# OATML/oatomobile

Hardware: AMD Instinct MI355X
Metric: RIPAgent.act() calls/sec (K=4, 128 plans, 200x200 BEV) (higher is better)
Workload: dtype bf16 encoder (bf16 storage, fp32 accumulate) + flow/search: fp32 accumulate, GRU/head contractions as two-term binary16 (22-bit) operands on f16 MFMA (the waypoint / bias terms as three-term, 33-bit operands); 1 GPU; BASELINE configs[2]: RIPAgent K=4 WCM, N=128 candidate plans, 10 Adam steps, 200x200x2 BEV, bf16 encoder + fp32 flow; models=4, candidates=128, bev_channels=2, parallelism=observation-parallel replicas x1 (no data-path collective)

## Files before the change

oatomobile_amd/csrc/encoder_bf16_tile.hip:

```cpp
#include <cstdio>

#include "encoder.h"
#include "flow.h"

namespace rip {

namespace {

using f32x4 = __attribute__((ext_vector_type(4))) float;
using f32x2 = __attribute__((ext_vector_type(2))) float;
using bf16x8 = __attribute__((ext_vector_type(8))) __bf16;
using bf16x2 = __attribute__((ext_vector_type(2))) __bf16;
using u32x4 = __attribute__((ext_vector_type(4))) unsigned int;
using u32x2 = __attribute__((ext_vector_type(2))) unsigned int;
typedef unsigned short bf16_t;

__device__ __forceinline__ bf16x8 as_bf16x8(u32x4 u) {
  union {
    u32x4 u;
    bf16x8 v;
  } c;
  c.u = u;
  return c.v;
}
__device__ __forceinline__ f32x2 bfpair(unsigned u) {
  f32x2 r;
  r.x = __uint_as_float(u << 16);
  r.y = __uint_as_float(u & 0xffff0000u);
  return r;
}
__device__ __forceinline__ unsigned pack_bf16(f32x2 v) {
  union {
    bf16x2 h;
    unsigned u;
  } c;
  c.h = __builtin_convertvector(v, bf16x2);
  return c.u;
}
__device__ __forceinline__ f32x2 relu6_2(f32x2 v) {
  return __builtin_elementwise_min(__builtin_elementwise_max(v, f32x2{0.f, 0.f}), f32x2{6.f, 6.f});
}

#ifndef RIP_TILE_ABL
#define RIP_TILE_ABL 0
#endif

#ifdef RIP_TILE_TICKS
__device__ unsigned long long g_tile_ticks[16];
#define TILE_TICK(slot_)                                            \
  do {                                                              \
    const unsigned long long now_ = __builtin_readcyclecounter();   \
    tk[slot_] += now_ - tlast;                                      \
    tlast = now_;                                                   \
  } while (0)
#else
#define TILE_TICK(slot_) do { } while (0)
#endif

constexpr int HC = 64;
constexpr int LD = HC + 8;

struct TileArgs {
  const bf16_t* x;
  bf16_t* y;
  const float* wbase;
  const bf16_t* whbase;
  size_t model_stride;
  int k0;
  size_t we_off, be_off, wd_off, bd_off, wp_off, bp_off;
  int B, HID, residual, G;
};

template <int HIN, int STRIDE, int G>
struct TileGeom {
  static constexpr int HOUT = STRIDE == 1 ? HIN : (HIN + 1) / 2;
  static constexpr int HWI = HIN * HIN, HWO = HOUT * HOUT;
  static constexpr int PW = HIN + 2;
  static constexpr int E_DUMP = G * HIN * PW;
  static constexpr int E_ROWS = E_DUMP + 1;
  static constexpr int D_ROWS = ((G * HWO + 15) / 16) * 16;
  static constexpr int TIN = (G * HWI + 63) / 64, TOUT = (G * HWO + 63) / 64;
  static constexpr size_t ED_BYTES = (size_t)2 * (E_ROWS + D_ROWS) * LD * sizeof(bf16_t);
  static constexpr size_t lds_bytes(int hid) { return ED_BYTES + (size_t)10 * hid * sizeof(float); }
};

template <int HIN, int STRIDE, int CIN, int COUT, int G, bool AEF, bool APF, int WCH = 1>
__global__ __launch_bounds__(512) void irb_tile_bf16_kernel(TileArgs a) {
  using Geo = TileGeom<HIN, STRIDE, G>;
  constexpr int HOUT = Geo::HOUT, HWI = Geo::HWI, HWO = Geo::HWO, PW = Geo::PW;
  constexpr int WP = 4 / WCH;
  constexpr int TIN = (Geo::TIN * 4 + WP - 1) / WP, TOUT = (Geo::TOUT * 4 + WP - 1) / WP;
  constexpr int KSX = CIN / 32, NCT = COUT / 16 / WCH, NHT = HC / 16 / WCH, NKP = HC / 32;
  static_assert((COUT / 16) % WCH == 0 && (HC / 16) % WCH == 0, "channel partitions");
  constexpr int NPT_IN = (G * HWI + 15) / 16, NPT_OUT = (G * HWO + 15) / 16;
  constexpr int CTG = NCT > 10 ? 10 : NCT;
  static_assert(NCT % CTG == 0 && (CTG == NCT || !APF), "projection passes");
  extern __shared__ __attribute__((aligned(16))) unsigned char smem_raw[];
  bf16_t* const Ebuf = reinterpret_cast<bf16_t*>(smem_raw);
  bf16_t* const Dbuf = Ebuf + (size_t)2 * Geo::E_ROWS * LD;
  float* const Tl = reinterpret_cast<float*>(smem_raw + Geo::ED_BYTES);
  const int tid = threadIdx.x, lane = tid & 63;
  const int w = __builtin_amdgcn_readfirstlane(tid >> 6);
  const int k = blockIdx.z;
  const int HID = a.HID;
  const int nch = HID / HC;
  const float* W = a.wbase + (size_t)(a.k0 + k) * a.model_stride;
  const bf16_t* Wh = a.whbase + (size_t)(a.k0 + k) * a.model_stride;
  const u32x4 zero4 = {0u, 0u, 0u, 0u};
  const int n_groups = (a.B + a.G - 1) / a.G;
  const int ng = (n_groups - 1 - (int)blockIdx.x) / (int)gridDim.x + 1;
  int img0 = 0, m_in = 0, m_out = 0;
  const bf16_t* xg = nullptr;
  bf16_t* yg = nullptr;
  auto enter_group = [&](int j) {
    img0 = ((int)blockIdx.x + j * (int)gridDim.x) * a.G;
    const int n_img = min(a.G, a.B - img0);
    m_in = n_img * HWI;
    m_out = n_img * HWO;
    xg = a.x + ((size_t)k * a.B + img0) * HWI * CIN;
    yg = a.y + ((size_t)k * a.B + img0) * HWO * COUT;
  };

#ifdef RIP_TILE_TICKS
  unsigned long long tk[10] = {0, 0, 0, 0, 0, 0, 0, 0, 0, 0};
  unsigned long long tlast = __builtin_readcyclecounter();
#endif
  if (!(RIP_TILE_ABL & 8))
    for (int e = tid; e < 2 * Geo::E_ROWS * LD / 8; e += 512) reinterpret_cast<u32x4*>(Ebuf)[e] = zero4;
  {
    const int HIDs = a.HID;
    const float* Wk = a.wbase + (size_t)(a.k0 + blockIdx.z) * a.model_stride;
    for (int e = tid; e < 9 * HIDs / 4; e += 512)
      reinterpret_cast<float4*>(Tl)[e] = *reinterpret_cast<const float4*>(Wk + a.wd_off + 4 * e);
    for (int e = tid; e < HIDs / 4; e += 512)
      reinterpret_cast<float4*>(Tl + 9 * HIDs)[e] = *reinterpret_cast<const float4*>(Wk + a.bd_off + 4 * e);
  }
  lds_barrier();
  TILE_TICK(0);

  if (w < 4) {
    const int n = lane & 15, q = lane >> 4;
    const int wpix = w / WCH, wch = w % WCH;
    const int ht0 = wch * NHT, ct0w = wch * NCT;
    u32x4 xb[TIN][KSX];
    int erow[TIN];
    f32x4 acc[TOUT][NCT];

    u32x4 ae[NHT][KSX], ap[CTG][NKP];
    float4 be[NHT];
    auto load_ae = [&](int c) {
      int n_ = n, q_ = q;
      asm volatile("" : "+v"(n_), "+v"(q_));
#pragma unroll
      for (int ht = 0; ht < NHT; ++ht) {
#pragma unroll
        for (int ks = 0; ks < KSX; ++ks)
          ae[ht][ks] = *reinterpret_cast<const u32x4*>(Wh + a.we_off + (size_t)(c * HC + 16 * (ht0 + ht) + n_) * CIN + 32 * ks + 8 * q_);
        be[ht] = *reinterpret_cast<const float4*>(W + a.be_off + c * HC + 16 * (ht0 + ht) + 4 * q_);
      }
    };
    auto load_ap = [&](int c, int ct0) {
      int n_ = n, q_ = q;
      asm volatile("" : "+v"(n_), "+v"(q_));
      const bf16_t* wp = Wh + a.wp_off + (size_t)(16 * (ct0w + ct0) + n_) * HID + c * HC + 8 * q_;
#pragma unroll
      for (int ct = 0; ct < CTG; ++ct)
#pragma unroll
        for (int ks = 0; ks < NKP; ++ks) ap[ct][ks] = *reinterpret_cast<const u32x4*>(wp + (size_t)16 * ct * HID + 32 * ks);
    };
    auto tile_on = [&](int t, int npt) { return !(WP * t + WP - 1 >= npt && wpix + WP * t >= npt); };
    auto expand = [&](int c) {
      bf16_t* E = Ebuf + (size_t)(c & 1) * Geo::E_ROWS * LD;
      if (!AEF && !((RIP_TILE_ABL & 32) && c > 0)) load_ae(c);
      f32x4 v[2][NHT];
      auto mm = [&](int t, f32x4(&o)[NHT]) {
#pragma unroll
        for (int ht = 0; ht < NHT; ++ht) o[ht] = f32x4{0.f, 0.f, 0.f, 0.f};
#pragma unroll
        for (int ks = 0; ks < KSX; ++ks)
#pragma unroll
          for (int ht = 0; ht < NHT; ++ht)
            o[ht] = __builtin_amdgcn_mfma_f32_16x16x32_bf16(as_bf16x8(ae[ht][ks]), as_bf16x8(xb[t][ks]), o[ht], 0, 0, 0);
      };
      auto epi = [&](int t, const f32x4(&o)[NHT]) {
#pragma unroll
        for (int ht = 0; ht < NHT; ++ht) {
          u32x2 w2;
          w2.x = pack_bf16(relu6_2(f32x2{o[ht][0] + be[ht].x, o[ht][1] + be[ht].y}));
          w2.y = pack_bf16(relu6_2(f32x2{o[ht][2] + be[ht].z, o[ht][3] + be[ht].w}));
          *reinterpret_cast<u32x2*>(E + (size_t)erow[t] * LD + 16 * (ht0 + ht) + 4 * q) = w2;
        }
      };
      if (tile_on(0, NPT_IN)) mm(0, v[0]);
#pragma unroll
      for (int t = 0; t < TIN; ++t) {
        if (t + 1 < TIN && tile_on(t + 1, NPT_IN)) mm(t + 1, v[(t + 1) & 1]);
        if (tile_on(t, NPT_IN)) epi(t, v[t & 1]);
      }
      if (AEF && c + 1 < nch && !(RIP_TILE_ABL & 32)) load_ae(c + 1);
    };
    auto project = [&](int c) {
      const bf16_t* D = Dbuf + (size_t)(c & 1) * Geo::D_ROWS * LD;
#pragma unroll
      for (int cg = 0; cg < NCT; cg += CTG) {
        if (!APF && !((RIP_TILE_ABL & 32) && c > 0)) load_ap(c, cg);
        u32x4 bv[2][NKP];
        auto rd = [&](int t, u32x4(&o)[NKP]) {
#pragma unroll
          for (int ks = 0; ks < NKP; ++ks)
            o[ks] = *reinterpret_cast<const u32x4*>(D + (size_t)(16 * (wpix + WP * t) + n) * LD + 32 * ks + 8 * q);
        };
        if (tile_on(0, NPT_OUT)) rd(0, bv[0]);
#pragma unroll
        for (int t = 0; t < TOUT; ++t) {
          if (t + 1 < TOUT && tile_on(t + 1, NPT_OUT)) rd(t + 1, bv[(t + 1) & 1]);
          if (!tile_on(t, NPT_OUT)) continue;
#pragma unroll
          for (int ks = 0; ks < NKP; ++ks)
#pragma unroll
            for (int ct = 0; ct < CTG; ++ct)
              acc[t][cg + ct] = __builtin_amdgcn_mfma_f32_16x16x32_bf16(as_bf16x8(ap[ct][ks]), as_bf16x8(bv[t & 1][ks]), acc[t][cg + ct], 0, 0, 0);
        }
      }
      if (APF && c + 1 < nch && !(RIP_TILE_ABL & 32)) load_ap(c + 1, 0);
    };
    const bool mx_on = !(RIP_TILE_ABL & 2);
#pragma unroll 1
    for (int j = 0; j < ng; ++j) {
    enter_group(j);
    int ng_ = n, qg_ = q;
    asm volatile("" : "+v"(ng_), "+v"(qg_));
#pragma unroll
    for (int t = 0; t < TIN; ++t) {
      const int px = 16 * (wpix + WP * t) + ng_;
#pragma unroll
      for (int ks = 0; ks < KSX; ++ks)
        xb[t][ks] = px < m_in ? *reinterpret_cast<const u32x4*>(xg + (size_t)px * CIN + 32 * ks + 8 * qg_) : zero4;
      const int g = px / HWI, r = px - g * HWI, iy = r / HIN, ix = r - iy * HIN;
      erow[t] = px < m_in ? g * HIN * PW + iy * PW + ix + 1 : Geo::E_DUMP;
    }
#pragma unroll
    for (int t = 0; t < TOUT; ++t)
#pragma unroll
      for (int ct = 0; ct < NCT; ++ct) acc[t][ct] = f32x4{0.f, 0.f, 0.f, 0.f};
    if (AEF) load_ae(0);
    if (APF) load_ap(0, 0);
    TILE_TICK(1);
#pragma unroll 1
    for (int s = 0; s < nch; ++s) {
      if (mx_on) expand(s);
      TILE_TICK(2);
      if (s >= 2 && mx_on) project(s - 2);
      TILE_TICK(3);
      lds_barrier();
      TILE_TICK(4);
    }
    float4 bpj[NCT];
    u32x2 rres[TOUT][NCT];
    int ne_ = n, qe_ = q;
    asm volatile("" : "+v"(ne_), "+v"(qe_));
#pragma unroll
    for (int ct = 0; ct < NCT; ++ct) bpj[ct] = *reinterpret_cast<const float4*>(W + a.bp_off + 16 * (ct0w + ct) + 4 * qe_);
#pragma unroll
    for (int t = 0; t < TOUT; ++t) {
      const int p = 16 * (wpix + WP * t) + ne_;
#pragma unroll
      for (int ct = 0; ct < NCT; ++ct)
        rres[t][ct] = (a.residual && p < m_out) ? *reinterpret_cast<const u32x2*>(xg + (size_t)p * CIN + 16 * (ct0w + ct) + 4 * qe_)
                                                : u32x2{0u, 0u};
    }
    TILE_TICK(5);
    if (nch >= 2 && mx_on) project(nch - 2);
    TILE_TICK(6);
    lds_barrier();
    TILE_TICK(7);
    if (mx_on) project(nch - 1);
    TILE_TICK(6);
    lds_barrier();
    TILE_TICK(7);
#pragma unroll
    for (int t = 0; t < TOUT; ++t) {
      const int p = 16 * (wpix + WP * t) + ne_;
      if (p >= m_out || (RIP_TILE_ABL & 16)) continue;
      if ((RIP_TILE_ABL & 64) && a.k0 >= 0) continue;
#pragma unroll
      for (int ct = 0; ct < NCT; ++ct) {
        f32x2 v0 = {acc[t][ct][0] + bpj[ct].x, acc[t][ct][1] + bpj[ct].y};
        f32x2 v1 = {acc[t][ct][2] + bpj[ct].z, acc[t][ct][3] + bpj[ct].w};
        v0 += bfpair(rres[t][ct].x);
        v1 += bfpair(rres[t][ct].y);
        u32x2 o;
        o.x = pack_bf16(v0);
        o.y = pack_bf16(v1);
        *reinterpret_cast<u32x2*>(yg + (size_t)p * COUT + 16 * (ct0w + ct) + 4 * qe_) = o;
      }
    }
    TILE_TICK(8);
    }
#ifdef RIP_TILE_TICKS
    if (tid == 0) {
#pragma unroll
      for (int i = 0; i < 9; ++i) atomicAdd(&g_tile_ticks[i], tk[i]);
      atomicAdd(&g_tile_ticks[9], 1ull);
    }
#endif
  } else {
    const int vt = tid - 256;
    const int c8 = vt & 7, dcol = (vt >> 3) % HOUT, dimg = (vt >> 3) / HOUT;
    const int dimg_c = dimg < G ? dimg : 0;
    const int e_off = (dimg_c * HIN * PW + dcol * STRIDE) * LD + 8 * c8;
    const int d_off = (dimg_c * HWO + dcol) * LD + 8 * c8;
    f32x2 wt[2][9][4], bd[2][4];
    auto load_taps = [&](int c, f32x2(&wt_)[9][4], f32x2(&bd_)[4]) {
      const float* wd = Tl + c * HC + 8 * c8;
#pragma unroll
      for (int t = 0; t < 9; ++t) {
        const float4 w0 = *reinterpret_cast<const float4*>(wd + (size_t)t * HID);
        const float4 w1 = *reinterpret_cast<const float4*>(wd + (size_t)t * HID + 4);
        wt_[t][0] = f32x2{w0.x, w0.y};
        wt_[t][1] = f32x2{w0.z, w0.w};
        wt_[t][2] = f32x2{w1.x, w1.y};
        wt_[t][3] = f32x2{w1.z, w1.w};
      }
      const float4 b0 = *reinterpret_cast<const float4*>(Tl + 9 * HID + c * HC + 8 * c8);
      const float4 b1 = *reinterpret_cast<const float4*>(Tl + 9 * HID + c * HC + 8 * c8 + 4);
      bd_[0] = f32x2{b0.x, b0.y};
      bd_[1] = f32x2{b0.z, b0.w};
      bd_[2] = f32x2{b1.x, b1.y};
      bd_[3] = f32x2{b1.z, b1.w};
    };
    auto depthwise = [&](const bf16_t* E, bf16_t* D, const f32x2(&wt_)[9][4], const f32x2(&bd_)[4]) {
      f32x2 sacc[HOUT][4];
#pragma unroll
      for (int iy = 0; iy < HIN; ++iy) {
        const bf16_t* r = E + e_off + iy * PW * LD;
        const u32x4 v0 = *reinterpret_cast<const u32x4*>(r);
        const u32x4 v1 = *reinterpret_cast<const u32x4*>(r + LD);
        const u32x4 v2 = *reinterpret_cast<const u32x4*>(r + 2 * LD);
        const f32x2 f[3][4] = {{bfpair(v0.x), bfpair(v0.y), bfpair(v0.z), bfpair(v0.w)},
                               {bfpair(v1.x), bfpair(v1.y), bfpair(v1.z), bfpair(v1.w)},
                               {bfpair(v2.x), bfpair(v2.y), bfpair(v2.z), bfpair(v2.w)}};
#pragma unroll
        for (int oy = 0; oy < HOUT; ++oy) {
          const int ky = iy - oy * STRIDE + 1;
          if (ky < 0 || ky > 2) continue;
          if (ky == 0 || (ky == 1 && oy * STRIDE - 1 < 0)) {
#pragma unroll
            for (int e = 0; e < 4; ++e) sacc[oy][e] = bd_[e];
          }
#pragma unroll
          for (int kx = 0; kx < 3; ++kx)
#pragma unroll
            for (int e = 0; e < 4; ++e) sacc[oy][e] = __builtin_elementwise_fma(f[kx][e], wt_[ky * 3 + kx][e], sacc[oy][e]);
          if (ky == 2 || iy == HIN - 1) {
            u32x4 o;
            o.x = pack_bf16(relu6_2(sacc[oy][0]));
            o.y = pack_bf16(relu6_2(sacc[oy][1]));
            o.z = pack_bf16(relu6_2(sacc[oy][2]));
            o.w = pack_bf16(relu6_2(sacc[oy][3]));
            *reinterpret_cast<u32x4*>(D + d_off + oy * HOUT * LD) = o;
          }
        }
      }
    };
#pragma unroll 1
    for (int j = 0; j < ng; ++j) {
    enter_group(j);
    const bool dw_on = dimg * HWI < m_in;
    load_taps(0, wt[0], bd[0]);
    TILE_TICK(1);
#pragma unroll 1
    for (int s = 0; s < nch + 2; s += 2) {
      if (s >= 1 && s <= nch && dw_on && !(RIP_TILE_ABL & 1))
        depthwise(Ebuf + (size_t)Geo::E_ROWS * LD, Dbuf + (size_t)Geo::D_ROWS * LD, wt[1], bd[1]);
      if (s + 1 < nch && !(RIP_TILE_ABL & 4)) load_taps(s + 1, wt[1], bd[1]);
      TILE_TICK(2);
      lds_barrier();
      TILE_TICK(3);
      if (s + 1 >= nch + 2) break;
      if (s + 1 <= nch && dw_on && !(RIP_TILE_ABL & 1)) depthwise(Ebuf, Dbuf, wt[0], bd[0]);
      if (s + 2 < nch && !(RIP_TILE_ABL & 4)) load_taps(s + 2, wt[0], bd[0]);
      TILE_TICK(2);
      lds_barrier();
      TILE_TICK(3);
    }
    }
#ifdef RIP_TILE_TICKS
    if (tid == 256) {
      atomicAdd(&g_tile_ticks[10], tk[2]);
      atomicAdd(&g_tile_ticks[11], tk[3]);
    }
#endif
  }
}

template <int HIN, int STRIDE, int CIN, int COUT, int GMAX, bool AEF, bool APF, int WCH = 1>
hipError_t launch_tile(TileArgs a, int kc, hipStream_t s) {
  using Geo = TileGeom<HIN, STRIDE, GMAX>;
  static_assert(GMAX * Geo::HOUT * 8 <= 256, "one depthwise thread per (observation, column, 8 channels)");
  int G = (int)(((long)a.B * kc + 255) / 256);
  if (G > GMAX) G = GMAX;
  if (G < 1) G = 1;
  a.G = G;
  static bool attr_set[64] = {};
  auto kern = irb_tile_bf16_kernel<HIN, STRIDE, CIN, COUT, GMAX, AEF, APF, WCH>;
  int dev = 0;
  if (hipGetDevice(&dev) != hipSuccess) return hipGetLastError();
  if (dev >= 0 && dev < 64 && !attr_set[dev]) {
    hipError_t e = hipFuncSetAttribute(reinterpret_cast<const void*>(kern), hipFuncAttributeMaxDynamicSharedMemorySize,
                                       (int)Geo::lds_bytes(6 * CIN));
    if (e != hipSuccess) return e;
    attr_set[dev] = true;
  }
  if (a.HID != 6 * CIN) return hipErrorInvalidValue;
  static_assert(Geo::lds_bytes(6 * CIN) <= 160 * 1024, "LDS budget");
  const int n_groups = (a.B + G - 1) / G;
  int gx = device_cu_count() / kc;
  if (gx < 1) gx = 1;
  if (gx > n_groups) gx = n_groups;
  note_kernel(dim3(gx, 1, kc), dim3(512), "irb_tile_bf16_kernel<%d,%d,%d,%d,%d,%s,%s,%d> G=%d", HIN, STRIDE, CIN, COUT,
              GMAX, AEF ? "true" : "false", APF ? "true" : "false", WCH, G);
  hipLaunchKernelGGL(kern, dim3(gx, 1, kc), dim3(512), Geo::lds_bytes(a.HID), s, a);
#ifdef RIP_TILE_TICKS
  {
    unsigned long long t[16];
    (void)hipDeviceSynchronize();
    (void)hipMemcpyFromSymbol(t, HIP_SYMBOL(g_tile_ticks), sizeof(t));
    const double n = t[9] > 0 ? (double)t[9] : 1.0, st = a.HID / HC;
    fprintf(stderr, "tile<%d,%d,%d,%d,G%d,%d> cycles per workgroup: prologue %.0f setup %.0f | per step (%d): expand %.0f project %.0f barrier %.0f | "
            "drain: requests %.0f projections 2 x %.0f barriers 2 x %.0f epilogue %.0f | vector wave per step: work %.0f barrier %.0f\n",
            HIN, STRIDE, CIN, COUT, G, WCH, t[0] / n, t[1] / n, (int)st, t[2] / n / st, t[3] / n / st, t[4] / n / st, t[5] / n, t[6] / n / 2,
            t[7] / n / 2, t[8] / n, t[10] / n / (st + 2), t[11] / n / (st + 2));
    unsigned long long z[16] = {};
    (void)hipMemcpyToSymbol(HIP_SYMBOL(g_tile_ticks), z, sizeof(z));
  }
#endif
  return hipGetLastError();
}

}

bool irb_tile_bf16_supported(const Layer* le, const Layer& ld, const Layer& lp, bool f17_layerwise) {
  if (le == nullptr) return false;
  const int cin = le->cin, hid = ld.cout, cout = lp.cout;
  if (hid != 6 * cin || hid % HC != 0) return false;
  if (ld.h_in == 7 && ld.stride == 1) return (cin == 64 && (cout == 64 || cout == 96)) || (cin == 96 && cout == 96);
  if (ld.h_in == 7 && ld.stride == 2) return cin == 96 && cout == 160;
  if (ld.h_in == 4 && ld.stride == 1) return cin == 160 && (cout == 160 || (!f17_layerwise && cout == 320));
  return false;
}

hipError_t launch_irb_tile_bf16(const Layer* le, const Layer& ld, const Layer& lp, const float* enc_w,
                                const unsigned short* enc_wh, size_t model_stride, int k0, int kc, int B,
                                const unsigned short* x, unsigned short* y, hipStream_t s) {
  TileArgs a;
  a.x = x;
  a.y = y;
  a.wbase = enc_w;
  a.whbase = enc_wh;
  a.model_stride = model_stride;
  a.k0 = k0;
  a.we_off = le->w_off;
  a.be_off = le->b_off;
  a.wd_off = ld.w_off;
  a.bd_off = ld.b_off;
  a.wp_off = lp.w_off;
  a.bp_off = lp.b_off;
  a.B = B;
  a.HID = ld.cout;
  a.residual = lp.residual;
  a.G = 1;
  const int cin = le->cin, cout = lp.cout;
  if (ld.h_in == 7 && ld.stride == 1) {
    if (cin == 64 && cout == 64) return launch_tile<7, 1, 64, 64, 4, true, true, 2>(a, kc, s);
    if (cin == 64 && cout == 96) return launch_tile<7, 1, 64, 96, 4, true, true, 2>(a, kc, s);
    if (cin == 96 && cout == 96) return launch_tile<7, 1, 96, 96, 4, false, false, 2>(a, kc, s);
  }
  if (ld.h_in == 7 && ld.stride == 2 && cin == 96 && cout == 160) return launch_tile<7, 2, 96, 160, 4, true, true, 2>(a, kc, s);
  if (ld.h_in == 4 && ld.stride == 1 && cin == 160) {
    if (cout == 160) return launch_tile<4, 1, 160, 160, 8, false, false, 2>(a, kc, s);
    if (cout == 320) return launch_tile<4, 1, 160, 320, 4, true, true, 4>(a, kc, s);
  }
  return hipErrorInvalidValue;
}

}
```

Baseline: 131,700 calls/s.

## Stage per-chunk encoder weights into LDS via async global_load_lds by idle waves

For the 96->96 and 160->160 inverted-residual tile kernels, the otherwise vector-only waves now issue direct global-to-LDS copies (global_load_lds) of expand/projection weights and depthwise taps for upcoming hidden chunks into double-buffered LDS sets. The matrix waves then read their operands from LDS instead of global memory, and the full-HID tap table is no longer preloaded. This is meant to hide weight-fetch latency behind compute and shrink the LDS footprint. In exchange it adds waitcnt/barrier coupling, and it lowers the group size (GS=6 instead of 8 for 160, GS=4 for 96), which may reduce the work done per workgroup.

Result: slower. 126,700 calls/s (-3.8%).

```diff
diff --git a/oatomobile_amd/csrc/encoder_bf16_tile.hip b/oatomobile_amd/csrc/encoder_bf16_tile.hip
--- a/oatomobile_amd/csrc/encoder_bf16_tile.hip
+++ b/oatomobile_amd/csrc/encoder_bf16_tile.hip
@@ -43,6 +43,9 @@
 
 #ifndef RIP_TILE_ABL
 #define RIP_TILE_ABL 0
+#endif
+#ifndef RIP_TILE_WST96
+#define RIP_TILE_WST96 1
 #endif
 
 #ifdef RIP_TILE_TICKS
@@ -84,21 +87,41 @@
   static constexpr size_t lds_bytes(int hid) { return ED_BYTES + (size_t)10 * hid * sizeof(float); }
 };
 
-template <int HIN, int STRIDE, int CIN, int COUT, int G, bool AEF, bool APF, int WCH = 1>
+template <int CIN, int COUT, int WST>
+struct StageGeom {
+  static constexpr int NFE = CIN / 8, NFP = COUT / 8;
+  static constexpr unsigned TP_OFF = 0, TP_BYTES = 10 * HC * sizeof(float);
+  static constexpr unsigned BE_OFF = TP_OFF + TP_BYTES, BE_BYTES = (WST & 1) ? HC * sizeof(float) : 0;
+  static constexpr unsigned WE_OFF = BE_OFF + BE_BYTES, WE_BYTES = (WST & 1) ? NFE * 1024 : 0;
+  static constexpr unsigned WP_OFF = WE_OFF + WE_BYTES, WP_BYTES = (WST & 2) ? NFP * 1024 : 0;
+  static constexpr unsigned SET_BYTES = WP_OFF + WP_BYTES;
+};
+template <int HIN, int STRIDE, int CIN, int COUT, int GS, int WST>
+constexpr size_t tile_lds_bytes() {
+  return WST ? TileGeom<HIN, STRIDE, GS>::ED_BYTES + 2 * (size_t)StageGeom<CIN, COUT, WST>::SET_BYTES
+             : TileGeom<HIN, STRIDE, GS>::lds_bytes(6 * CIN);
+}
+typedef __attribute__((address_space(3))) void* lds_ptr_t;
+
+template <int HIN, int STRIDE, int CIN, int COUT, int G, bool AEF, bool APF, int WCH = 1, int WST = 0, int GS = G>
 __global__ __launch_bounds__(512) void irb_tile_bf16_kernel(TileArgs a) {
-  using Geo = TileGeom<HIN, STRIDE, G>;
+  using Geo = TileGeom<HIN, STRIDE, GS>;
+  using Stg = StageGeom<CIN, COUT, WST>;
+  static_assert(GS <= G && !((WST & 1) && AEF) && !((WST & 2) && APF), "staged operands are not requested into registers ahead");
+  static_assert(Stg::NFE % 4 == 0 && Stg::NFP % 4 == 0 && HC == 64, "pieces per vector wave");
   constexpr int HOUT = Geo::HOUT, HWI = Geo::HWI, HWO = Geo::HWO, PW = Geo::PW;
   constexpr int WP = 4 / WCH;
   constexpr int TIN = (Geo::TIN * 4 + WP - 1) / WP, TOUT = (Geo::TOUT * 4 + WP - 1) / WP;
   constexpr int KSX = CIN / 32, NCT = COUT / 16 / WCH, NHT = HC / 16 / WCH, NKP = HC / 32;
   static_assert((COUT / 16) % WCH == 0 && (HC / 16) % WCH == 0, "channel partitions");
-  constexpr int NPT_IN = (G * HWI + 15) / 16, NPT_OUT = (G * HWO + 15) / 16;
+  constexpr int NPT_IN = (GS * HWI + 15) / 16, NPT_OUT = (GS * HWO + 15) / 16;
   constexpr int CTG = NCT > 10 ? 10 : NCT;
   static_assert(NCT % CTG == 0 && (CTG == NCT || !APF), "projection passes");
   extern __shared__ __attribute__((aligned(16))) unsigned char smem_raw[];
   bf16_t* const Ebuf = reinterpret_cast<bf16_t*>(smem_raw);
   bf16_t* const Dbuf = Ebuf + (size_t)2 * Geo::E_ROWS * LD;
   float* const Tl = reinterpret_cast<float*>(smem_raw + Geo::ED_BYTES);
+  unsigned char* const Sg = smem_raw + Geo::ED_BYTES;
   const int tid = threadIdx.x, lane = tid & 63;
   const int w = __builtin_amdgcn_readfirstlane(tid >> 6);
   const int k = blockIdx.z;
@@ -127,7 +150,58 @@
 #endif
   if (!(RIP_TILE_ABL & 8))
     for (int e = tid; e < 2 * Geo::E_ROWS * LD / 8; e += 512) reinterpret_cast<u32x4*>(Ebuf)[e] = zero4;
-  {
+  const unsigned sg_lds = (unsigned)(size_t)(lds_ptr_t)Sg;
+  auto dma16 = [&](const void* src, unsigned lds_byte) {
+    asm volatile("s_mov_b32 m0, %0\n\ts_nop 0\n\tglobal_load_lds_dwordx4 %1, off" ::"s"(lds_byte), "v"(src) : "memory");
+  };
+  auto dma4 = [&](const void* src, unsigned lds_byte) {
+    asm volatile("s_mov_b32 m0, %0\n\ts_nop 0\n\tglobal_load_lds_dword %1, off" ::"s"(lds_byte), "v"(src) : "memory");
+  };
+  auto copy_we = [&](int c) {
+    const unsigned set = sg_lds + (unsigned)(c & 1) * Stg::SET_BYTES;
+    const int v = w - 4, n = lane & 15, q = lane >> 4;
+    const bf16_t* src = Wh + a.we_off + (size_t)(c * HC + n) * CIN + 8 * q;
+#pragma unroll
+    for (int f = 0; f < Stg::NFE / 4; ++f) {
+      const int p = v + 4 * f, ht = p / (CIN / 32), ks = p - ht * (CIN / 32);
+      dma16(src + (size_t)16 * ht * CIN + 32 * ks, set + Stg::WE_OFF + (unsigned)p * 1024u);
+    }
+    if (v == 0) dma4(W + a.be_off + c * HC + lane, set + Stg::BE_OFF);
+  };
+  auto copy_wp = [&](int c) {
+    const unsigned set = sg_lds + (unsigned)(c & 1) * Stg::SET_BYTES;
+    const int v = w - 4, n = lane & 15, q = lane >> 4;
+    const bf16_t* src = Wh + a.wp_off + (size_t)n * HID + c * HC + 8 * q;
+#pragma unroll
+    for (int f = 0; f < Stg::NFP / 4; ++f) {
+      const int p = v + 4 * f, ct = p >> 1, ks = p & 1;
+      dma16(src + (size_t)16 * ct * HID + 32 * ks, set + Stg::WP_OFF + (unsigned)p * 1024u);
+    }
+  };
+  auto copy_tp = [&](int c) {
+    const unsigned set = sg_lds + (unsigned)(c & 1) * Stg::SET_BYTES + Stg::TP_OFF;
+    const int v = w - 4;
+    if (v < 2) dma16(W + a.wd_off + (size_t)(4 * v + (lane >> 4)) * HID + c * HC + 4 * (lane & 15), set + (unsigned)v * 1024u);
+    else if (v == 2) dma4(W + a.wd_off + (size_t)8 * HID + c * HC + lane, set + 2048u);
+    else dma4(W + a.bd_off + c * HC + lane, set + 2304u);
+  };
+  auto stage = [&](int s, bool more) {
+    if (WST & 1) {
+      if (s + 1 < nch) copy_we(s + 1);
+      else if (s == nch + 1 && more) copy_we(0);
+    }
+    if ((WST & 2) && s >= 1 && s <= nch) copy_wp(s - 1);
+    if (s + 2 < nch) copy_tp(s + 2);
+    else if (s >= nch && more) copy_tp(s - nch);
+  };
+  if (WST) {
+    if (w >= 4) {
+      if (WST & 1) copy_we(0);
+      copy_tp(0);
+      copy_tp(1);
+      asm volatile("s_waitcnt vmcnt(0)" ::: "memory");
+    }
+  } else {
     const int HIDs = a.HID;
     const float* Wk = a.wbase + (size_t)(a.k0 + blockIdx.z) * a.model_stride;
     for (int e = tid; e < 9 * HIDs / 4; e += 512)
@@ -149,6 +223,17 @@
     u32x4 ae[NHT][KSX], ap[CTG][NKP];
     float4 be[NHT];
     auto load_ae = [&](int c) {
+      if constexpr ((WST & 1) != 0) {
+        const unsigned char* set = Sg + (size_t)(c & 1) * Stg::SET_BYTES;
+#pragma unroll
+        for (int ht = 0; ht < NHT; ++ht) {
+#pragma unroll
+          for (int ks = 0; ks < KSX; ++ks)
+            ae[ht][ks] = *reinterpret_cast<const u32x4*>(set + Stg::WE_OFF + ((ht0 + ht) * KSX + ks) * 1024 + lane * 16);
+          be[ht] = *reinterpret_cast<const float4*>(set + Stg::BE_OFF + (16 * (ht0 + ht) + 4 * q) * sizeof(float));
+        }
+        return;
+      }
       int n_ = n, q_ = q;
       asm volatile("" : "+v"(n_), "+v"(q_));
 #pragma unroll
@@ -160,6 +245,15 @@
       }
     };
     auto load_ap = [&](int c, int ct0) {
+      if constexpr ((WST & 2) != 0) {
+        const unsigned char* set = Sg + (size_t)(c & 1) * Stg::SET_BYTES;
+#pragma unroll
+        for (int ct = 0; ct < CTG; ++ct)
+#pragma unroll
+          for (int ks = 0; ks < NKP; ++ks)
+            ap[ct][ks] = *reinterpret_cast<const u32x4*>(set + Stg::WP_OFF + ((ct0w + ct0 + ct) * NKP + ks) * 1024 + lane * 16);
+        return;
+      }
       int n_ = n, q_ = q;
       asm volatile("" : "+v"(n_), "+v"(q_));
       const bf16_t* wp = Wh + a.wp_off + (size_t)(16 * (ct0w + ct0) + n_) * HID + c * HC + 8 * q_;
@@ -225,6 +319,7 @@
       if (APF && c + 1 < nch && !(RIP_TILE_ABL & 32)) load_ap(c + 1, 0);
     };
     const bool mx_on = !(RIP_TILE_ABL & 2);
+    if (WST) lds_barrier();
 #pragma unroll 1
     for (int j = 0; j < ng; ++j) {
     enter_group(j);
@@ -307,23 +402,25 @@
   } else {
     const int vt = tid - 256;
     const int c8 = vt & 7, dcol = (vt >> 3) % HOUT, dimg = (vt >> 3) / HOUT;
-    const int dimg_c = dimg < G ? dimg : 0;
+    const int dimg_c = dimg < GS ? dimg : 0;
     const int e_off = (dimg_c * HIN * PW + dcol * STRIDE) * LD + 8 * c8;
     const int d_off = (dimg_c * HWO + dcol) * LD + 8 * c8;
     f32x2 wt[2][9][4], bd[2][4];
     auto load_taps = [&](int c, f32x2(&wt_)[9][4], f32x2(&bd_)[4]) {
-      const float* wd = Tl + c * HC + 8 * c8;
+      const float* tl = WST ? reinterpret_cast<const float*>(Sg + (size_t)(c & 1) * Stg::SET_BYTES + Stg::TP_OFF) : Tl + c * HC;
+      const int ts = WST ? HC : HID;
+      const float* wd = tl + 8 * c8;
 #pragma unroll
       for (int t = 0; t < 9; ++t) {
-        const float4 w0 = *reinterpret_cast<const float4*>(wd + (size_t)t * HID);
-        const float4 w1 = *reinterpret_cast<const float4*>(wd + (size_t)t * HID + 4);
+        const float4 w0 = *reinterpret_cast<const float4*>(wd + (size_t)t * ts);
+        const float4 w1 = *reinterpret_cast<const float4*>(wd + (size_t)t * ts + 4);
         wt_[t][0] = f32x2{w0.x, w0.y};
         wt_[t][1] = f32x2{w0.z, w0.w};
         wt_[t][2] = f32x2{w1.x, w1.y};
         wt_[t][3] = f32x2{w1.z, w1.w};
       }
-      const float4 b0 = *reinterpret_cast<const float4*>(Tl + 9 * HID + c * HC + 8 * c8);
-      const float4 b1 = *reinterpret_cast<const float4*>(Tl + 9 * HID + c * HC + 8 * c8 + 4);
+      const float4 b0 = *reinterpret_cast<const float4*>(wd + (size_t)9 * ts);
+      const float4 b1 = *reinterpret_cast<const float4*>(wd + (size_t)9 * ts + 4);
       bd_[0] = f32x2{b0.x, b0.y};
       bd_[1] = f32x2{b0.z, b0.w};
       bd_[2] = f32x2{b1.x, b1.y};
@@ -363,24 +460,47 @@
         }
       }
     };
+    auto landed = [&]() {
+      if (WST) {
+        asm volatile("s_waitcnt vmcnt(0)" ::: "memory");
+        TILE_TICK(5);
+      }
+    };
+    if (WST) {
+      load_taps(0, wt[0], bd[0]);
+      lds_barrier();
+    }
 #pragma unroll 1
     for (int j = 0; j < ng; ++j) {
     enter_group(j);
     const bool dw_on = dimg * HWI < m_in;
-    load_taps(0, wt[0], bd[0]);
+    const bool more = j + 1 < ng;
+    if (!WST) load_taps(0, wt[0], bd[0]);
     TILE_TICK(1);
 #pragma unroll 1
     for (int s = 0; s < nch + 2; s += 2) {
+      if (WST) {
+        stage(s, more);
+        TILE_TICK(4);
+      }
       if (s >= 1 && s <= nch && dw_on && !(RIP_TILE_ABL & 1))
         depthwise(Ebuf + (size_t)Geo::E_ROWS * LD, Dbuf + (size_t)Geo::D_ROWS * LD, wt[1], bd[1]);
       if (s + 1 < nch && !(RIP_TILE_ABL & 4)) load_taps(s + 1, wt[1], bd[1]);
+      if (WST && s == nch + 1 && more) load_taps(0, wt[0], bd[0]);
       TILE_TICK(2);
+      landed();
       lds_barrier();
       TILE_TICK(3);
       if (s + 1 >= nch + 2) break;
+      if (WST) {
+        stage(s + 1, more);
+        TILE_TICK(4);
+      }
       if (s + 1 <= nch && dw_on && !(RIP_TILE_ABL & 1)) depthwise(Ebuf, Dbuf, wt[0], bd[0]);
       if (s + 2 < nch && !(RIP_TILE_ABL & 4)) load_taps(s + 2, wt[0], bd[0]);
+      if (WST && s + 1 == nch + 1 && more) load_taps(0, wt[0], bd[0]);
       TILE_TICK(2);
+      landed();
       lds_barrier();
       TILE_TICK(3);
     }
@@ -389,38 +509,40 @@
     if (tid == 256) {
       atomicAdd(&g_tile_ticks[10], tk[2]);
       atomicAdd(&g_tile_ticks[11], tk[3]);
+      atomicAdd(&g_tile_ticks[12], tk[4]);
+      atomicAdd(&g_tile_ticks[13], tk[5]);
     }
 #endif
   }
 }
 
-template <int HIN, int STRIDE, int CIN, int COUT, int GMAX, bool AEF, bool APF, int WCH = 1>
+template <int HIN, int STRIDE, int CIN, int COUT, int GMAX, bool AEF, bool APF, int WCH = 1, int WST = 0, int GS = GMAX>
 hipError_t launch_tile(TileArgs a, int kc, hipStream_t s) {
-  using Geo = TileGeom<HIN, STRIDE, GMAX>;
+  using Geo = TileGeom<HIN, STRIDE, GS>;
   static_assert(GMAX * Geo::HOUT * 8 <= 256, "one depthwise thread per (observation, column, 8 channels)");
+  constexpr size_t LDS_BYTES = tile_lds_bytes<HIN, STRIDE, CIN, COUT, GS, WST>();
   int G = (int)(((long)a.B * kc + 255) / 256);
-  if (G > GMAX) G = GMAX;
+  if (G > GS) G = GS;
   if (G < 1) G = 1;
   a.G = G;
   static bool attr_set[64] = {};
-  auto kern = irb_tile_bf16_kernel<HIN, STRIDE, CIN, COUT, GMAX, AEF, APF, WCH>;
+  auto kern = irb_tile_bf16_kernel<HIN, STRIDE, CIN, COUT, GMAX, AEF, APF, WCH, WST, GS>;
   int dev = 0;
   if (hipGetDevice(&dev) != hipSuccess) return hipGetLastError();
   if (dev >= 0 && dev < 64 && !attr_set[dev]) {
-    hipError_t e = hipFuncSetAttribute(reinterpret_cast<const void*>(kern), hipFuncAttributeMaxDynamicSharedMemorySize,
-                                       (int)Geo::lds_bytes(6 * CIN));
+    hipError_t e = hipFuncSetAttribute(reinterpret_cast<const void*>(kern), hipFuncAttributeMaxDynamicSharedMemorySize, (int)LDS_BYTES);
     if (e != hipSuccess) return e;
     attr_set[dev] = true;
   }
   if (a.HID != 6 * CIN) return hipErrorInvalidValue;
-  static_assert(Geo::lds_bytes(6 * CIN) <= 160 * 1024, "LDS budget");
+  static_assert(LDS_BYTES <= 160 * 1024, "LDS budget");
   const int n_groups = (a.B + G - 1) / G;
   int gx = device_cu_count() / kc;
   if (gx < 1) gx = 1;
   if (gx > n_groups) gx = n_groups;
   note_kernel(dim3(gx, 1, kc), dim3(512), "irb_tile_bf16_kernel<%d,%d,%d,%d,%d,%s,%s,%d> G=%d", HIN, STRIDE, CIN, COUT,
               GMAX, AEF ? "true" : "false", APF ? "true" : "false", WCH, G);
-  hipLaunchKernelGGL(kern, dim3(gx, 1, kc), dim3(512), Geo::lds_bytes(a.HID), s, a);
+  hipLaunchKernelGGL(kern, dim3(gx, 1, kc), dim3(512), LDS_BYTES, s, a);
 #ifdef RIP_TILE_TICKS
   {
     unsigned long long t[16];
@@ -428,9 +550,9 @@
     (void)hipMemcpyFromSymbol(t, HIP_SYMBOL(g_tile_ticks), sizeof(t));
     const double n = t[9] > 0 ? (double)t[9] : 1.0, st = a.HID / HC;
     fprintf(stderr, "tile<%d,%d,%d,%d,G%d,%d> cycles per workgroup: prologue %.0f setup %.0f | per step (%d): expand %.0f project %.0f barrier %.0f | "
-            "drain: requests %.0f projections 2 x %.0f barriers 2 x %.0f epilogue %.0f | vector wave per step: work %.0f barrier %.0f\n",
+            "drain: requests %.0f projections 2 x %.0f barriers 2 x %.0f epilogue %.0f | vector wave per step: work %.0f barrier %.0f copies: issue %.0f wait %.0f\n",
             HIN, STRIDE, CIN, COUT, G, WCH, t[0] / n, t[1] / n, (int)st, t[2] / n / st, t[3] / n / st, t[4] / n / st, t[5] / n, t[6] / n / 2,
-            t[7] / n / 2, t[8] / n, t[10] / n / (st + 2), t[11] / n / (st + 2));
+            t[7] / n / 2, t[8] / n, t[10] / n / (st + 2), t[11] / n / (st + 2), t[12] / n / (st + 2), t[13] / n / (st + 2));
     unsigned long long z[16] = {};
     (void)hipMemcpyToSymbol(HIP_SYMBOL(g_tile_ticks), z, sizeof(z));
   }
@@ -474,11 +596,20 @@
   if (ld.h_in == 7 && ld.stride == 1) {
     if (cin == 64 && cout == 64) return launch_tile<7, 1, 64, 64, 4, true, true, 2>(a, kc, s);
     if (cin == 64 && cout == 96) return launch_tile<7, 1, 64, 96, 4, true, true, 2>(a, kc, s);
+#ifdef RIP_TILE_NOSTAGE
     if (cin == 96 && cout == 96) return launch_tile<7, 1, 96, 96, 4, false, false, 2>(a, kc, s);
+#else
+    if (cin == 96 && cout == 96)
+      return launch_tile<7, 1, 96, 96, 4, false, false, 2, RIP_TILE_WST96, RIP_TILE_WST96 == 3 ? 3 : 4>(a, kc, s);
+#endif
   }
   if (ld.h_in == 7 && ld.stride == 2 && cin == 96 && cout == 160) return launch_tile<7, 2, 96, 160, 4, true, true, 2>(a, kc, s);
   if (ld.h_in == 4 && ld.stride == 1 && cin == 160) {
+#ifdef RIP_TILE_NOSTAGE
     if (cout == 160) return launch_tile<4, 1, 160, 160, 8, false, false, 2>(a, kc, s);
+#else
+    if (cout == 160) return launch_tile<4, 1, 160, 160, 8, false, false, 2, 3, 6>(a, kc, s);
+#endif
     if (cout == 320) return launch_tile<4, 1, 160, 320, 4, true, true, 4>(a, kc, s);
   }
   return hipErrorInvalidValue;
```
